# TaihuLight/Lol

Hardware: AMD Instinct MI355X
Metric: cyclotomic poly-muls/sec (CRT·pointwise·CRT⁻¹), batched; bit-exact vs CT (higher is better)
Workload: dtype u64

## Files before the change

lol_amd/csrc/pow2_impl.h:

```cpp
#pragma once
#include <hip/hip_runtime.h>

#include <atomic>
#include <mutex>
#include <type_traits>
#include <utility>

#include "kernels.h"
#include "zq_dev.h"

namespace lolhip {


constexpr int R = 4;
constexpr int E = 1 << R;
#ifndef LOLHIP_LEVEL_PARTS
#define LOLHIP_LEVEL_PARTS 4
#endif

#ifdef LOLHIP_STAMPS
static __device__ unsigned long long* g_stamp_buf = nullptr;
#define LH_STAMP(i) do { unsigned long long t_; asm volatile("s_memtime %0\n\ts_waitcnt lgkmcnt(0)" : "=s"(t_) :: "memory"); \
    if (g_stamp_buf && (threadIdx.x & 63) == 0) g_stamp_buf[((size_t)blockIdx.x * (blockDim.x >> 6) + (threadIdx.x >> 6)) * 32 + (i)] = t_; } while (0)
#else
// ... 53 lines not shown
    j += len;
  }
  return r;
}
template <Lay A, int I>
__device__ __forceinline__ int xthr_run(int tau) {
  constexpr LayRuns r = lay_runs(A);
  if constexpr (I < r.n) return (((tau >> r.src[I]) & ((1 << r.len[I]) - 1)) << r.dst[I]) | xthr_run<A, I + 1>(tau);
  else return 0;
}
template <Lay A>
__device__ __forceinline__ int xthr(int tau) { return xthr_run<A, 0>(tau); }

template <Lay A> struct LayTab {
  int xr[E];
  constexpr LayTab() : xr{} { for (int e = 0; e < E; ++e) xr[e] = xreg(A, e); }
};
template <Lay A> inline constexpr LayTab<A> lay_tab{};

constexpr int lpad(int x) { return x + (x >> 4); }

template <int AR> using VT = std::conditional_t<AR >= 2, u32, u64>;

struct QK {
  u64 q, nq, q2, nq2, q4, nq4;
  template <bool UNIFORM>
  __device__ __forceinline__ QK(const ModCtx& mc, std::bool_constant<UNIFORM> u) : QK(mc.q, u) {}
  template <bool UNIFORM>
  __device__ __forceinline__ QK(u64 q_, std::bool_constant<UNIFORM>) : q(q_), nq(0 - q_), q2(2 * q_), nq2(0 - 2 * q_), q4(4 * q_), nq4(0 - 4 * q_) {
    if constexpr (UNIFORM) asm volatile("" : "+s"(nq), "+s"(nq2), "+s"(nq4));
    else asm volatile("" : "+v"(nq), "+v"(nq2), "+v"(nq4));
  }
};
struct QK32 {
  u32 q, q2, mu;
  u32 r, rp, nqinv;
  template <bool UNIFORM>
  __device__ __forceinline__ QK32(const ModCtx& mc, std::bool_constant<UNIFORM>)
      : q((u32)mc.q), q2(2 * (u32)mc.q), mu((u32)(mc.mu >> 32)), r(mc.r32), rp(mc.r32p), nqinv((u32)mc.nqinv) {}
};
template <int AR> using QKT = std::conditional_t<AR >= 2, QK32, QK>;

__device__ __forceinline__ u32 csub32(u32 x, u32 m) { return min(x, x - m); }
__device__ __forceinline__ u32 shoup32(u32 y, u32 w, u32 wp, u32 q) { return w * y - __umulhi(wp, y) * q; }

#ifndef LOLHIP_PAIR_BFLY
#define LOLHIP_PAIR_BFLY 0
#endif
__device__ __forceinline__ u64 pair_of(u32 lo) { typedef u32 u32p __attribute__((ext_vector_type(2))); u32p t; t.x = lo; return __builtin_bit_cast(u64, t); }
template <bool WS>
__device__ __forceinline__ void fwd_pair(u32& X, u32& Y, u32 x, u32 w, u32 wp, u32 q, u32 q2) {
  const u64 xp = pair_of(x), q2p = (u64)q2;
  const u32 nq = 0u - q;
  u64 Xn, Z, Yn, cy; u32 Q;
#define LH_FWD_PAIR(WC)                                                                                     \
  asm("v_mul_hi_u32 %[Q], %[wp], %[yl]\n\t"                                                                  \
      "v_mad_u64_u32 %[Xn], %[cy], %[w], %[yl], %[X]\n\t"                                                    \
      "v_lshl_add_u64 %[Z], %[X], 1, %[q2]\n\t"                                                              \
      "v_mad_u64_u32 %[Xn], %[cy], %[Q], %[nq], %[Xn]"                                                        \
      : [Q] "=&v"(Q), [Xn] "=&v"(Xn), [Z] "=&v"(Z), [cy] "=&s"(cy)                                            \
      : [wp] WC(wp), [yl] "v"(Y), [w] WC(w), [X] "v"(xp), [q2] "s"(q2p), [nq] "s"(nq))
  if constexpr (WS) { LH_FWD_PAIR("s"); } else { LH_FWD_PAIR("v"); }
#undef LH_FWD_PAIR
  asm("v_mad_u64_u32 %[Yn], %[cy], %[xl], -1, %[Z]" : [Yn] "=v"(Yn), [cy] "=s"(cy) : [xl] "v"((u32)Xn), [Z] "v"(Z));
  X = (u32)Xn; Y = (u32)Yn;
}
template <bool WS>
__device__ __forceinline__ u32 shoup_pair(u32 d, u32 w, u32 wp, u32 q) {
  const u32 nq = 0u - q;
  const u32 Q = __umulhi(wp, d);
  u64 T, Yn, cy;
#define LH_SH_PAIR(WC)                                                                                      \
  asm("v_mad_u64_u32 %[T], %[cy], %[w], %[d], 0\n\t"                                                         \
      "v_mad_u64_u32 %[Yn], %[cy], %[Q], %[nq], %[T]"                                                         \
      : [T] "=&v"(T), [Yn] "=&v"(Yn), [cy] "=&s"(cy) : [w] WC(w), [d] "v"(d), [Q] "v"(Q), [nq] "s"(nq))
  if constexpr (WS) { LH_SH_PAIR("s"); } else { LH_SH_PAIR("v"); }
#undef LH_SH_PAIR
  return (u32)Yn;
}

template <int AR, bool WS = false, bool L1 = false>
__device__ __forceinline__ void bfly_fwd(VT<AR>& X, VT<AR>& Y, VT<AR> w, VT<AR> wp, const QKT<AR>& k) {
  if constexpr (AR == 3) {
    const u32 x = csub32(X, k.q);
    const u32 t = csub32(shoup32(Y, w, wp, k.q), k.q);
    X = x + t;
    Y = x - t + k.q;
  } else if constexpr (AR == 2) {
    const u32 x = csub32(X, k.q2);
#if LOLHIP_PAIR_BFLY
    fwd_pair<WS>(X, Y, x, w, wp, k.q, k.q2);
#else
    const u32 t = shoup32(Y, w, wp, k.q);
    X = x + t;
    Y = x - t + k.q2;
#endif
  } else if constexpr (AR == 4) {
#if LOLHIP_PAIR_BFLY
    fwd_pair<WS>(X, Y, X, w, wp, k.q, k.q2);
#else
    const u32 t = shoup32(Y, w, wp, k.q);
    const u32 x = X;
    X = x + t;
    Y = x - t + k.q2;
#endif
  } else if constexpr (AR == 1) {
#ifdef LH_ABL_NO_FWD_CSUB
    const u64 x = X;
#else
    const u64 x = L1 ? X : csubn(X, k.nq4);
#endif
    const u64 xn = shoup_acc<WS>(Y, w, wp, k.nq, x);
    const u64 z = shl1_add64u(x, k.q4);
    X = xn;
    Y = z - xn;
  } else {
    const u64 x = csub(X, k.q2);
    const u64 t = shoup_lazy(Y, w, wp, k.q);
    X = x + t;
    Y = x - t + k.q2;
  }
}
template <int AR, bool WS = false>
__device__ __forceinline__ void bfly_inv(VT<AR>& X, VT<AR>& Y, VT<AR> w, VT<AR> wp, const QKT<AR>& k) {
  if constexpr (AR == 3) {
    const u32 s = X + Y;
    const u32 d = X - Y + k.q;
    X = csub32(s, k.q);
    Y = csub32(shoup32(d, w, wp, k.q), k.q);
  } else if constexpr (AR == 2 || AR == 4) {
    const u32 s = X + Y;
    const u32 d = X - Y + k.q2;
    X = csub32(s, k.q2);
#if LOLHIP_PAIR_BFLY
    Y = shoup_pair<WS>(d, w, wp, k.q);
#else
    Y = shoup32(d, w, wp, k.q);
#endif
  } else if constexpr (AR == 1) {
    const u64 s = add64(X, Y);
    const u64 d = add64u(X, k.q4) - Y;
    X = csubn(s, k.nq4);
    Y = shoup_acc<WS>(d, w, wp, k.nq, 0);
  } else {
    const u64 s = X + Y;
    const u64 d = X - Y + k.q2;
    X = csub(s, k.q2);
    Y = shoup_lazy(d, w, wp, k.q);
  }
}
template <int AR, bool WS = false>
__device__ __forceinline__ void bfly_inv_last(VT<AR>& X, VT<AR>& Y, VT<AR> w, VT<AR> wp, VT<AR> s0, VT<AR> s1, const QKT<AR>& k) {
  if constexpr (AR == 3) {
    const u32 s = X + Y;
    const u32 d = X - Y + k.q;
    X = csub32(shoup32(s, s0, s1, k.q), k.q);
    Y = csub32(shoup32(d, w, wp, k.q), k.q);
  } else if constexpr (AR == 2 || AR == 4) {
    const u32 s = X + Y;
    const u32 d = X - Y + k.q2;
    X = shoup32(s, s0, s1, k.q);
    Y = shoup32(d, w, wp, k.q);
  } else if constexpr (AR == 1) {
    const u64 s = add64(X, Y);
    const u64 d = add64u(X, k.q4) - Y;
    X = shoup_acc<WS>(s, s0, s1, k.nq, 0);
    Y = shoup_acc<WS>(d, w, wp, k.nq, 0);
  } else {
    const u64 s = X + Y;
    const u64 d = X - Y + k.q2;
    X = shoup_lazy(s, s0, s1, k.q);
    Y = shoup_lazy(d, w, wp, k.q);
  }
}
template <int AR> __device__ __forceinline__ VT<AR> canon_fwd(VT<AR> v, const QKT<AR>& k) {
  if constexpr (AR == 3) return csub32(v, k.q);
  else if constexpr (AR == 2) return csub32(csub32(v, k.q2), k.q);
  else if constexpr (AR == 4) return csub32(v - __umulhi(v, k.mu) * k.q, k.q);
  else {
    if constexpr (AR == 1) v = csubn(v, k.nq4);
    return csubn(csubn(v, k.nq2), k.nq);
  }
}
template <int AR> __device__ __forceinline__ VT<AR> canon_inv(VT<AR> v, const QKT<AR>& k) {
  if constexpr (AR == 3) return v;
  else if constexpr (AR == 2 || AR == 4) return csub32(v, k.q);
  else {
    if constexpr (AR == 1) v = csubn(v, k.nq2);
    return csubn(v, k.nq);
  }
}
template <int AR> __device__ __forceinline__ VT<AR> from_i64(i64 x, const QKT<AR>& k) {
  if constexpr (AR >= 2) return (u32)x + (k.q & (u32)(x >> 63));
  else return canon_in(x, k.q);
}
template <int AR> __device__ __forceinline__ VT<AR> from_i64_fwd(i64 x, const QKT<AR>& k) {
  if constexpr (AR == 1) return add64u((u64)x, k.q);
  else if constexpr (AR >= 2) return (u32)x + k.q;
  else return from_i64<AR>(x, k);
}
template <int AR> __device__ __forceinline__ VT<AR> from_i64_inv(i64 x, const QKT<AR>& k) {
  if constexpr (AR == 1) return add64u((u64)x, k.q2);
  else if constexpr (AR == 2 || AR == 4) return (u32)x + k.q;
  else return from_i64<AR>(x, k);
}
template <int AR> __device__ __forceinline__ VT<AR> park_fwd(VT<AR> v, const QKT<AR>& k) {
  if constexpr (AR >= 2) return csub32(shoup32(v, k.r, k.rp, k.q), k.q);
  else if constexpr (AR == 1) return csubn(csubn(v, k.nq4), k.nq2);
  else return canon_fwd<AR>(v, k);
}
template <int AR> __device__ __forceinline__ VT<AR> pmul(VT<AR> a, VT<AR> b, const ModCtx& mc, const QKT<AR>& k) {
  if constexpr (AR >= 2) {
    const u64 x = (u64)a * b;
    const u32 m = (u32)x * k.nqinv;
    const u32 t = (u32)((x + (u64)m * k.q) >> 32);
    if constexpr (AR == 3) return csub32(t, k.q);
    else return t;
  } else if constexpr (AR == 1) {
#ifdef LOLHIP_ABL_PMUL
    return a + b;
#endif
    const unsigned __int128 T = (unsigned __int128)a * b;
    const u64 lo = (u64)T;
    return (u64)(T >> 64) + __umul64hi(lo * mc.nqinv, mc.q) + (lo != 0);
  } else {
    return mulmod(a, canon_fwd<0>(b, k), mc);
  }
}

typedef u32 u32x2 __attribute__((ext_vector_type(2)));
typedef u32 u32x4 __attribute__((ext_vector_type(4)));
typedef __amdgpu_buffer_rsrc_t rsrc_t;

__device__ __forceinline__ void load_tw(rsrc_t tw, u32 voff, u32 const_idx, u64& w, u64& wp) {
// ... 142 lines not shown
        load_tw(INV ? tw.inv : tw.fwd, voff, (u32)cidx, t.w[ord], t.wp[ord]);
      }
    }
    ++ord;
  }
}
template <int NT, typename V>
__device__ __forceinline__ void tw_fill_lds(V* dst, rsrc_t src, u32 comp, int n, int tau) {
  const int cnt = (n < TWL_HI ? n : TWL_HI) - TWL_LO;
  for (int i = tau; i < cnt; i += NT) {
    if constexpr (sizeof(V) == 8) {
      const u32x4 r = __builtin_amdgcn_raw_buffer_load_b128(src, comp + (u32)(TWL_LO + i) * 16u, 0, 0);
      *reinterpret_cast<u32x4*>(dst + 2 * i) = r;
    } else {
      const u32x2 r = __builtin_amdgcn_raw_buffer_load_b64(src, comp + (u32)(TWL_LO + i) * 8u, 0, 0);
      *reinterpret_cast<u32x2*>(dst + 2 * i) = r;
    }
  }
}
#ifndef LOLHIP_WS
#define LOLHIP_WS 1
#endif
template <int AR, bool INV, Lay A, int K, int HALF = -1>
__device__ __forceinline__ void level(VT<AR> (&v)[E], const LevelTwT<VT<AR>>& t, const TwCtxT<VT<AR>>& tw, const QKT<AR>& qk) {
  constexpr int beta = A.reg[K];
#ifdef LOLHIP_ABL_NO_BFLY
#pragma unroll
  for (int s = 0; s < 8; ++s) asm volatile("" :: "v"(t.w[s]), "v"(t.wp[s]));
  return;
#endif
  int ordb = -1;
#pragma unroll
  for (int e = 0; e < E; ++e) {
    if (e & (1 << K)) continue;
    ++ordb;
    if (HALF >= 0 && ordb / (8 / LOLHIP_LEVEL_PARTS) != HALF) continue;
    const int s = level_tab<A, K>.slot[e];
    constexpr bool WU = LOLHIP_WS && (A.ntb + R >= 10);
    if constexpr (!INV) bfly_fwd<AR, WU && tw_uniform<A, K>(), beta == 0>(v[e], v[e | (1 << K)], t.w[s], t.wp[s], qk);
    else if constexpr (beta == 0) bfly_inv_last<AR, WU>(v[e], v[e | (1 << K)], tw.l1w, tw.l1wp, tw.sc0, tw.sc1, qk);
    else bfly_inv<AR, WU && tw_uniform<A, K>()>(v[e], v[e | (1 << K)], t.w[s], t.wp[s], qk);
  }
}

template <int TB, int RK>
__device__ __forceinline__ void lane_swap(u32 (&v)[E]) {
  static_assert(TB == 4 || TB == 5, "only lane bits 4 and 5 have swap instructions");
// ... 86 lines not shown
  }
  static constexpr int G_K0 = R - (L - 10);
  static constexpr Lay io() {
    if (W16) {
      if (L < 10) { int thr[12] = {1, 2, 3, 4, 5, 6, 7, 8, 9, 10, 11, 12}; return lay_make(L, 0, L - 3, L - 2, L - 1, thr); }
      int thr[12] = {1, 2, 3, 4, 5, 6, 10, 11, 12, 13, 14, 15};
      return lay_make(L, 0, 7, 8, 9, thr);
    }
    if (L < 10) return lay_std(L, L - R);
    int thr[12] = {0, 1, 2, 3, 4, 5, 10, 11, 12, 13, 14, 15};
    return lay_make(L, 6, 7, 8, 9, thr);
  }
  static constexpr Lay final_layout() { return HAS_G ? g() : wave_end(); }
};

template <int AR, bool INV, Lay A, int K0, int K1 = R>
__device__ __forceinline__ void fetch4(LevelTwT<VT<AR>> (&t)[R], const TwCtxT<VT<AR>>& tw, int xt) {
  if constexpr (K0 <= 0 && K1 > 0) tw_fetch<INV, A, 0>(t[0], tw, xt);
  if constexpr (K0 <= 1 && K1 > 1) tw_fetch<INV, A, 1>(t[1], tw, xt);
  if constexpr (K0 <= 2 && K1 > 2) tw_fetch<INV, A, 2>(t[2], tw, xt);
  if constexpr (K0 <= 3 && K1 > 3) tw_fetch<INV, A, 3>(t[3], tw, xt);
}
template <int AR, bool INV, Lay A, int K>
__device__ __forceinline__ void level_jit(VT<AR> (&v)[E], const TwCtxT<VT<AR>>& tw, int xt, const QKT<AR>& qk) {
  using LevelTw = LevelTwT<VT<AR>>;
  if constexpr (tw_distinct(A, K) == 8 && sizeof(VT<AR>) == 8) {
    [&]<int... PART>(std::integer_sequence<int, PART...>) {
      (([&] { LevelTw t; tw_fetch<INV, A, K, PART>(t, tw, xt); level<AR, INV, A, K, PART>(v, t, tw, qk); }()), ...);
    }(std::make_integer_sequence<int, LOLHIP_LEVEL_PARTS>{});
  } else {
    LevelTw t; tw_fetch<INV, A, K>(t, tw, xt); level<AR, INV, A, K>(v, t, tw, qk);
  }
}
template <int AR, Lay A, int K0, int K1 = R>
__device__ __forceinline__ void levels4_jit(VT<AR> (&v)[E], const TwCtxT<VT<AR>>& tw, int xt, const QKT<AR>& qk) {
  if constexpr (K0 <= 0 && K1 > 0) level_jit<AR, false, A, 0>(v, tw, xt, qk);
  if constexpr (K0 <= 1 && K1 > 1) level_jit<AR, false, A, 1>(v, tw, xt, qk);
  if constexpr (K0 <= 2 && K1 > 2) level_jit<AR, false, A, 2>(v, tw, xt, qk);
  if constexpr (K0 <= 3 && K1 > 3) level_jit<AR, false, A, 3>(v, tw, xt, qk);
}
template <int AR, bool INV, Lay A, int K0, int K1 = R>
__device__ __forceinline__ void levels4(VT<AR> (&v)[E], const LevelTwT<VT<AR>> (&t)[R], const TwCtxT<VT<AR>>& tw, const QKT<AR>& qk) {
  if constexpr (!INV) {
    if constexpr (K0 <= 0 && K1 > 0) level<AR, false, A, 0>(v, t[0], tw, qk);
    if constexpr (K0 <= 1 && K1 > 1) level<AR, false, A, 1>(v, t[1], tw, qk);
    if constexpr (K0 <= 2 && K1 > 2) level<AR, false, A, 2>(v, t[2], tw, qk);
    if constexpr (K0 <= 3 && K1 > 3) level<AR, false, A, 3>(v, t[3], tw, qk);
  } else {
    if constexpr (K0 <= 3 && K1 > 3) level<AR, true, A, 3>(v, t[3], tw, qk);
    if constexpr (K0 <= 2 && K1 > 2) level<AR, true, A, 2>(v, t[2], tw, qk);
    if constexpr (K0 <= 1 && K1 > 1) level<AR, true, A, 1>(v, t[1], tw, qk);
    if constexpr (K0 <= 0 && K1 > 0) level<AR, true, A, 0>(v, t[0], tw, qk);
  }
}

__device__ __forceinline__ int fresh(int x) {
  asm volatile("" : "+v"(x));
  return x;
}

struct NoTop {};
template <int AR, int L, Lay PREV, int SB = 0, bool LEAN = false, bool W16 = false, typename TOP = NoTop, bool TRUNC = false>
__device__ __forceinline__ void fwd_transform(VT<AR> (&v)[E], VT<AR>* lds, const TwCtxT<VT<AR>>& tw, int tau_in, const QKT<AR>& qk,
                                              TOP* pre = nullptr) {
  constexpr bool PRE = !std::is_same_v<TOP, NoTop>;
  using LevelTw = LevelTwT<VT<AR>>;
  using S = Sched<L, W16>;
  static_assert(!TRUNC || (L >= 11 && !PRE), "the truncated forward transform needs the G layout");
  constexpr int GK1 = TRUNC ? 2 : R;
  constexpr bool L10 = !(TRUNC && L == 11);
  {
    constexpr Lay A = S::w0();
    const int tau = fresh(tau_in);
    if constexpr (S::HAS_G && !lay_eq(PREV, A)) __syncthreads();
    transpose_put<PREV, A, false>(v, lds, tau);
    if constexpr (LEAN) {
      transpose_get<PREV, A, false>(v, lds, tau);
      levels4_jit<AR, A, 0>(v, tw, xthr<A>(tau), qk);
    } else {
      LevelTw t[R];
      fetch4<AR, false, A, 0>(t, tw, xthr<A>(tau));
      transpose_get<PREV, A, false>(v, lds, tau);
      LH_STAMP(SB + 2);
      levels4<AR, false, A, 0>(v, t, tw, qk);
      LH_STAMP(SB + 3);
    }
// ... 39 lines not shown
    const int tau = fresh(tau_in);
    transpose_put<S::wave_end(), A, false>(v, lds, tau);
    if constexpr (PRE) {
      transpose_get<S::wave_end(), A, true>(v, lds, tau);
      LH_STAMP(SB + 7);
      pre->wait_g();
      levels4<AR, false, A, S::G_K0>(v, pre->g, tw, qk);
      LH_STAMP(SB + 8);
    } else if constexpr (LEAN) {
      transpose_get<S::wave_end(), A, true>(v, lds, tau);
      levels4_jit<AR, A, S::G_K0, GK1>(v, tw, xthr<A>(tau), qk);
    } else {
      LevelTw t[R];
      fetch4<AR, false, A, S::G_K0, GK1>(t, tw, xthr<A>(tau));
      transpose_get<S::wave_end(), A, true>(v, lds, tau);
      LH_STAMP(SB + 7);
      levels4<AR, false, A, S::G_K0, GK1>(v, t, tw, qk);
      LH_STAMP(SB + 8);
    }
  }
}

template <int AR, int L, Lay NEXT, bool W16 = false, bool TRUNC = false>
__device__ __forceinline__ void inv_transform(VT<AR> (&v)[E], VT<AR>* lds, const TwCtxT<VT<AR>>& tw, int tau_in, const QKT<AR>& qk) {
  using LevelTw = LevelTwT<VT<AR>>;
  using S = Sched<L, W16>;
  static_assert(!TRUNC || L >= 11, "the truncated inverse transform needs the G layout");
  constexpr int GK1 = TRUNC ? 2 : R;
  constexpr bool L10 = !(TRUNC && L == 11);
  if constexpr (S::HAS_G) {
    constexpr Lay A = S::g();
    const int tau = fresh(tau_in);
    LevelTw t[R];
    fetch4<AR, true, A, S::G_K0, GK1>(t, tw, xthr<A>(tau));
    levels4<AR, true, A, S::G_K0, GK1>(v, t, tw, qk);
    transpose_put<A, S::wave_end(), true>(v, lds, tau);
  }
  if constexpr (S::HAS_W1) {
    constexpr Lay A = S::w1();
    const int tau = fresh(tau_in);
    const int xt = xthr<A>(tau);
    LevelTw ua, ub, t[R];
    if constexpr (S::NSWAP >= 2 && L10) tw_fetch<true, S::w1b(), 2>(ub, tw, xthr<S::w1b()>(tau));
    if constexpr (S::NSWAP >= 1) tw_fetch<true, S::w1a(), 3>(ua, tw, xthr<S::w1a()>(tau));
    if constexpr (S::NSWAP == 0) fetch4<AR, true, A, S::W1_K0>(t, tw, xt);
    if constexpr (S::HAS_G) transpose_get<S::g(), S::wave_end(), true>(v, lds, tau);
    if constexpr (S::NSWAP >= 2) { if constexpr (L10) level<AR, true, S::w1b(), 2>(v, ub, tw, qk); lane_swap<5, 2>(v); }
// ... 52 lines not shown
        [y2l] "v"(lo32(y[2])), [y2h] "v"(hi32(y[2])), [y3l] "v"(lo32(y[3])), [y3h] "v"(hi32(y[3])));
}
__device__ __forceinline__ u64 dot4_redc(const u64 (&x)[4], const u64 (&y)[4], const ModCtx& mc) {
  u64 A, B1, B2, C;
  dot4_cols(x, y, A, B1, B2, C);
  const u64 u = (u64)hi32(C) + lo32(B1) + lo32(B2);
  const u64 lo = ((u64)lo32(u) << 32) | lo32(C);
  const u64 hi = A + hi32(B1) + hi32(B2) + hi32(u);
  return hi + __umul64hi(lo * mc.nqinv, mc.q) + (lo != 0);
}
template <Lay G>
__device__ __forceinline__ void pow2_base4(u64 (&v)[E], const u64 (&va)[E], const TwCtxT<u64>& tw, int xt, const ModCtx& mc, const QK& qk) {
  LevelTwT<u64> z;
  tw_fetch<false, G, 1>(z, tw, xt);
#pragma unroll
  for (int g = 0; g < 4; ++g) {
    constexpr int EK[4] = {0, 8, 4, 12};
    u64 zw = z.w[level_tab<G, 1>.slot[g & 1]], zwp = z.wp[level_tab<G, 1>.slot[g & 1]];
    if (g & 2) { zw = qk.q - zw; zwp = ~zwp; }
    u64 a[4], y[4];
#pragma unroll
    for (int k = 0; k < 4; ++k) {
      a[k] = va[g | EK[k]];
      y[k] = csubn(csubn(v[g | EK[k]], qk.nq4), qk.nq2);
    }
#pragma unroll
    for (int k = 3; k >= 0; --k) {
      u64 x[4], w[4];
#pragma unroll
      for (int i = 0; i < 4; ++i) { x[i] = a[i]; w[i] = y[(k - i) & 3]; }
      v[g | EK[k]] = dot4_redc(x, w, mc);
      asm volatile("" : "+v"(v[g | EK[k]]));
      if (k) y[k] = csubn(shoup_acc<false>(y[k], zw, zwp, qk.nq, 0), qk.nq2);
    }
  }
}

constexpr int pow2_threads(int L) { return (1 << (L - R)) >= 256 ? (1 << (L - R)) : 256; }

template <int L, int MODE, int AR, bool T1 = false, bool TR = false>
__global__ void __launch_bounds__(pow2_threads(L), AR >= 2 ? 8 : 4)
k_pow2(i64* y, const i64* a_in, const i64* b_in, i64 B, int T,
       const VT<AR>* __restrict__ tw_fwd, const VT<AR>* __restrict__ tw_inv, const VT<AR>* __restrict__ scale,
       const ModCtx* __restrict__ mod, int xcd_map) {
  using S = Sched<L, T1>;
  using V = VT<AR>;
  static_assert(!TR || (MODE == 2 && AR == 1 && L >= 11), "the truncated route is the 61-bit fused poly-mul's");
  constexpr int n = 1 << L;
  constexpr int NT = 1 << (L - R);
  constexpr int PPW = NT >= 256 ? 1 : 256 / NT;
  constexpr int LDSW = n + n / 16 + twl_words(n);
  constexpr u32 TWB = 2 * sizeof(V);
  extern __shared__ __attribute__((aligned(16))) unsigned char smem[];
  V* lds = reinterpret_cast<V*>(smem) + (threadIdx.x / NT) * LDSW;
  V* lds_tw = lds + n + n / 16;
  const int tau = threadIdx.x % NT;
  if constexpr (T1) T = 1;

  const i64 item0 = (i64)blockIdx.x * PPW;
  const int slot = (PPW == 1) ? 0 : (int)(threadIdx.x / NT);
  const i64 item = item0 + slot;
  i64 b, b0; int t;
  if (xcd_map) { i64 g = item / (8 * (i64)T); int r = (int)(item % (8 * T)); b = g * 8 + (r & 7); t = r >> 3; b0 = b; }
  else { b = item / T; t = (int)(item % T); b0 = item0 / T; }
  if constexpr (T1) { b = item; t = 0; b0 = item0; }

  if constexpr (NT >= 64) {
    t = __builtin_amdgcn_readfirstlane(t);
    b = (i64)(((u64)(u32)__builtin_amdgcn_readfirstlane((int)(b >> 32)) << 32) | (u32)__builtin_amdgcn_readfirstlane((int)b));
  }
  b0 = (i64)(((u64)(u32)__builtin_amdgcn_readfirstlane((int)(b0 >> 32)) << 32) | (u32)__builtin_amdgcn_readfirstlane((int)b0));
  const QKT<AR> qk(mod[t], std::bool_constant<(NT >= 64 || T1)>{});
  const u64 win = (u64)(B - b0) * n * T * 8;
  const u32 wbytes = win > 0xFFFFFFFFull ? 0xFFFFFFFFu : (u32)win;
  const size_t wbase = (size_t)b0 * n * T;
  const rsrc_t ry = __builtin_amdgcn_make_buffer_rsrc((void*)(y + wbase), 0, wbytes, 0x00020000);
  const rsrc_t ra = __builtin_amdgcn_make_buffer_rsrc((void*)(a_in + (MODE == 2 ? wbase : 0)), 0, MODE == 2 ? wbytes : 0, 0x00020000);
  const rsrc_t rb = __builtin_amdgcn_make_buffer_rsrc((void*)(b_in + (MODE == 2 ? wbase : 0)), 0, MODE == 2 ? wbytes : 0, 0x00020000);
  TwCtxT<V> tw;
  tw.fwd = __builtin_amdgcn_make_buffer_rsrc((void*)tw_fwd, 0, (u32)T * n * TWB, 0x00020000);
  tw.inv = __builtin_amdgcn_make_buffer_rsrc((void*)tw_inv, 0, (u32)T * n * TWB, 0x00020000);
  tw.comp = (u32)t * (u32)n * TWB;
  tw.pf = tw_fwd + (size_t)t * n * 2;
  tw.pi = tw_inv + (size_t)t * n * 2;
  tw.lds_tw = lds_tw;
  if constexpr (L >= TWL_MIN_L) tw_fill_lds<NT>(lds_tw, (MODE == 1) ? tw.inv : tw.fwd, tw.comp, n, tau);
  constexpr int SC = (MODE == 2 && AR == 1) ? 4 : 0;
  const V* scp = TR ? scale + (size_t)T * 8 + (size_t)t * 4 : scale + (size_t)t * 8 + SC;
  tw.sc0 = scp[0];
  tw.sc1 = scp[1];
  tw.l1w = scp[2];
  tw.l1wp = scp[3];

  constexpr Lay LIO = S::io();
  constexpr Lay LFIN = S::final_layout();
  const u32 uT8 = (u32)T * 8u;
  const u32 pofs = ((u32)(b - b0) * (u32)n * (u32)T + (u32)t) * 8u;
  const u32 off_io = pofs + (u32)xthr<LIO>(tau) * uT8;
  const u32 off_fin = pofs + (u32)xthr<LFIN>(tau) * uT8;

  V v[E];
  LH_STAMP(0);
#ifdef LOLHIP_STAMPS
  if (g_stamp_buf && (threadIdx.x & 63) == 0) {
    unsigned hwid, xcc;
    asm volatile("s_getreg_b32 %0, hwreg(HW_REG_HW_ID)" : "=s"(hwid));
    asm volatile("s_getreg_b32 %0, hwreg(HW_REG_XCC_ID)" : "=s"(xcc));
    g_stamp_buf[((size_t)blockIdx.x * (blockDim.x >> 6) + (threadIdx.x >> 6)) * 32 + 30] = ((unsigned long long)xcc << 32) | hwid;
  }
#endif
  if constexpr (MODE == 0 || MODE == 2) {
    const rsrc_t src = (MODE == 2) ? ra : ry;
    load_poly<LIO, T1>(src, off_io, uT8, [&](int e, u64 x) { v[e] = from_i64_fwd<AR>((i64)x, qk); });
    LH_STAMP(1);
    fwd_transform<AR, L, LIO, 0, false, T1, NoTop, TR>(v, lds, tw, tau, qk);
    if constexpr (MODE == 0) LH_STAMP(20);
  }
  if constexpr (MODE == 2) {
    V va[E];
#pragma unroll
    for (int e = 0; e < E; ++e) {
      va[e] = park_fwd<AR>(v[e], qk);
      if constexpr (TR) asm volatile("" : "+v"(va[e]));
    }
    LH_STAMP(9);
    const bool square = (a_in == b_in);
    if (!square) {
      u64 raw[E];
      load_poly<LIO, T1>(rb, off_io, uT8, [&](int e, u64 x) { raw[e] = x; });
      __builtin_amdgcn_sched_barrier(0);
#pragma unroll
      for (int e = 0; e < E; ++e) v[e] = from_i64_fwd<AR>((i64)raw[e], qk);
      LH_STAMP(11);
      fwd_transform<AR, L, LIO, 10, true, T1, NoTop, TR>(v, lds, tw, tau, qk);
    }
    LH_STAMP(19);
    const ModCtx mc = mod[t];
    if constexpr (TR) {
      pow2_base4<LFIN>(v, va, tw, xthr<LFIN>(fresh(tau)), mc, qk);
    } else {
#pragma unroll
      for (int e = 0; e < E; ++e) v[e] = pmul<AR>(va[e], (AR < 2 && square) ? va[e] : v[e], mc, qk);
    }
    LH_STAMP(22);
  }
  if constexpr (MODE == 2 && L >= TWL_MIN_L) {
    if constexpr (L > 10) __syncthreads();
    tw_fill_lds<NT>(lds_tw, tw.inv, tw.comp, n, tau);
  }
  if constexpr (MODE == 1) {
    load_poly<LFIN, T1>(ry, off_fin, uT8, [&](int e, u64 x) { v[e] = from_i64_inv<AR>((i64)x, qk); });
  }
  if constexpr (MODE == 0) {
    store_poly<LFIN, T1>(ry, off_fin, uT8, [&](int e) { return (u64)canon_fwd<AR>(v[e], qk); });
    LH_STAMP(21);
  } else {
    LH_STAMP(23);
    inv_transform<AR, L, LIO, T1, TR>(v, lds, tw, tau, qk);
    LH_STAMP(24);
    store_poly<LIO, T1>(ry, off_io, uT8, [&](int e) { return (u64)canon_inv<AR>(v[e], qk); });
    LH_STAMP(25);
  }
}

constexpr int MAX_DEV = 64;
struct KernelDev { std::atomic<int> state{0}; };
inline std::mutex& kernel_dev_mutex() { static std::mutex m; return m; }
template <typename Setup>
static hipError_t kernel_dev_setup(KernelDev (&tab)[MAX_DEV], Setup&& setup) {
  int dev = -1;
  hipError_t e = hipGetDevice(&dev);
  if (e != hipSuccess) return e;
  if (dev < 0 || dev >= MAX_DEV) return hipErrorInvalidDevice;
  KernelDev& d = tab[dev];
  if (d.state.load(std::memory_order_acquire) != 2) {
    std::lock_guard<std::mutex> g(kernel_dev_mutex());
    if (d.state.load(std::memory_order_relaxed) != 2) {
      e = setup();
      if (e != hipSuccess) return e;
      d.state.store(2, std::memory_order_release);
// ... 63 lines not shown
```

lol_amd/csrc/zq_dev.h:

```cpp
#pragma once
#include <stdint.h>

#if defined(__HIPCC__)
#include <hip/hip_runtime.h>
#define LH_HD __host__ __device__ __forceinline__
#define LH_D __device__ __forceinline__
#else
#define LH_HD inline
#define LH_D inline
#endif

namespace lolhip {

typedef uint64_t u64;
typedef uint32_t u32;
typedef int64_t i64;

struct ModCtx {
  u64 q;
  u64 d;
  u64 v;
  u32 s;
  u32 r32;
  u64 mu;
// ... 50 lines not shown

#ifndef LOLHIP_ASM_MAD
#define LOLHIP_ASM_MAD 3
#endif
LH_D u64 mad64(u32 a, u32 b, u64 c) {
#if LOLHIP_ASM_MAD
  u64 d, carry;
  asm("v_mad_u64_u32 %0, %1, %2, %3, %4" : "=v"(d), "=s"(carry) : "v"(a), "v"(b), "v"(c));
  return d;
#else
  return (u64)a * (u64)b + c;
#endif
}
LH_D u64 add64(u64 a, u64 b) { return a + b; }
LH_D u64 shl1_add64(u64 a, u64 b) { return (a << 1) + b; }
LH_D u64 add64u(u64 a, u64 b_uniform) { return a + b_uniform; }
LH_D u64 shl1_add64u(u64 a, u64 b_uniform) { return (a << 1) + b_uniform; }
LH_D u32 lo32(u64 x) { return (u32)x; }
LH_D u32 hi32(u64 x) { return (u32)(x >> 32); }

LH_D u64 csubn(u64 x, u64 negm) {
  u64 t = add64u(x, negm);
  return ((int)hi32(t) < 0) ? x : t;
}

template <bool WS = false>
LH_D u64 shoup_acc(u64 y, u64 w, u64 wp, u64 nq, u64 init) {
#if LOLHIP_ASM_MAD == 4
  u64 t = init, h, sj;
  asm("v_mad_u64_u32 v[120:121], vcc, %[wph], %[ylo], 0\n\t"
      "v_mad_u64_u32 v[120:121], vcc, %[wpl], %[yhi], v[120:121]\n\t"
      "v_mad_u64_u32 %[t], %[sj], %[wl], %[ylo], %[t]\n\t"
      "v_mad_u64_u32 %[h], %[sj], %[wl], %[yhi], 0\n\t"
      "v_mad_u64_u32 %[h], %[sj], %[wh], %[ylo], %[h]\n\t"
      "v_mov_b32 v122, v121\n\t"
      "v_cndmask_b32_e64 v123, 0, 1, vcc\n\t"
      "v_mad_u64_u32 v[118:119], %[sj], %[wph], %[yhi], v[122:123]\n\t"
      "v_mad_u64_u32 %[t], %[sj], v118, %[nql], %[t]\n\t"
      "v_mad_u64_u32 %[h], %[sj], v118, %[nqh], %[h]\n\t"
      "v_mad_u64_u32 %[h], %[sj], v119, %[nql], %[h]"
      : [t] "+v"(t), [h] "=&v"(h), [sj] "=&s"(sj)
      : [wph] "v"(hi32(wp)), [wpl] "v"(lo32(wp)), [ylo] "v"(lo32(y)), [yhi] "v"(hi32(y)),
        [wl] "v"(lo32(w)), [wh] "v"(hi32(w)), [nql] "s"(lo32(nq)), [nqh] "s"(hi32(nq))
      : "vcc", "v118", "v119", "v120", "v121", "v122", "v123");
  u32 th = hi32(t) + lo32(h);
  asm("" : "+v"(th));
// ... 32 lines not shown
  if constexpr (WS) { LH_SHOUP_BLOCKS(LH_WC_S); } else { LH_SHOUP_BLOCKS(LH_WC_V); }
#undef LH_SHOUP_BLOCKS
#undef LH_WC_V
#undef LH_WC_S
  u32 th = hi32(t) + lo32(h);
  asm("" : "+v"(th));
  return ((u64)th << 32) | lo32(t);
#else
  const u32 ah = __umulhi(hi32(wp), lo32(y));
  const u32 bh = __umulhi(lo32(wp), hi32(y));
  const u64 Q = mad64(bh, 1u, mad64(hi32(wp), hi32(y), (u64)ah));
  u64 t = mad64(lo32(w), lo32(y), init);
  t = mad64(lo32(Q), lo32(nq), t);
  u64 h = mad64(lo32(w), hi32(y), 0);
  h = mad64(hi32(w), lo32(y), h);
  h = mad64(lo32(Q), hi32(nq), h);
  h = mad64(hi32(Q), lo32(nq), h);
  u32 th = hi32(t) + lo32(h);
  asm("" : "+v"(th));
  return ((u64)th << 32) | lo32(t);
#endif
}

LH_D u64 rem128(u64 x1, u64 x0, const ModCtx& c) {
  u64 u1 = (x1 << c.s) | (x0 >> (64 - c.s));
  u64 u0 = x0 << c.s;
  unsigned __int128 qq = (unsigned __int128)c.v * u1 + (((unsigned __int128)u1 << 64) | u0);
  u64 q1 = (u64)(qq >> 64) + 1, q0 = (u64)qq;
  u64 r = u0 - q1 * c.d;
  if (r > q0) r += c.d;
  if (r >= c.d) r -= c.d;
  return r >> c.s;
}

LH_D u64 mulmod(u64 a, u64 b, const ModCtx& c) {
  unsigned __int128 z = (unsigned __int128)a * b;
  return rem128((u64)(z >> 64), (u64)z, c);
}

LH_D u64 reduce128(u64 x1, u64 x0, const ModCtx& c) {
  u64 r1 = rem128(0, x1, c);
  return rem128(r1, x0, c);
}

LH_D u64 addmod(u64 a, u64 b, u64 q) { u64 s = a + b; return s >= q ? s - q : s; }
LH_D u64 submod(u64 a, u64 b, u64 q) { return a >= b ? a - b : a + q - b; }
// ... 5 lines not shown
```

Before: 9.260 million.

## Use exec-masked conditional subtracts and defer per-modulus loads in tight mode

Adds csubx variants that perform 64-bit conditional subtraction with v_cmpx plus an exec-masked add, replacing the add/compare/select sequence in the radix-2 butterflies, canonicalisation and park steps when the modulus constants are wave-uniform. One of them is fused into the Shoup multiply asm block. For a small-thread-count pointwise mode, a new TIGHT path keeps per-lane constants unlaundered and defers loading inverse twiddle pointers and scale factors until the inverse transform, to cut live registers across the forward transform and pointwise stage. The cost is exec-mask manipulation with an s_nop pad and more template plumbing through auto-typed parameters.

```diff
diff --git a/lol_amd/csrc/pow2_impl.h b/lol_amd/csrc/pow2_impl.h
--- a/lol_amd/csrc/pow2_impl.h
+++ b/lol_amd/csrc/pow2_impl.h
@@ -99,16 +99,28 @@
 
 template <int AR> using VT = std::conditional_t<AR >= 2, u32, u64>;
 
-struct QK {
+template <bool UNIFORM, bool LAUNDER = true>
+struct QKx {
+  static constexpr bool uniform = UNIFORM;
   u64 q, nq, q2, nq2, q4, nq4;
-  template <bool UNIFORM>
-  __device__ __forceinline__ QK(const ModCtx& mc, std::bool_constant<UNIFORM> u) : QK(mc.q, u) {}
-  template <bool UNIFORM>
-  __device__ __forceinline__ QK(u64 q_, std::bool_constant<UNIFORM>) : q(q_), nq(0 - q_), q2(2 * q_), nq2(0 - 2 * q_), q4(4 * q_), nq4(0 - 4 * q_) {
+  __device__ __forceinline__ QKx(const ModCtx& mc, std::bool_constant<UNIFORM> u) : QKx(mc.q, u) {}
+  __device__ __forceinline__ QKx(u64 q_, std::bool_constant<UNIFORM>) : q(q_), nq(0 - q_), q2(2 * q_), nq2(0 - 2 * q_), q4(4 * q_), nq4(0 - 4 * q_) {
+    static_assert(LAUNDER || !UNIFORM, "only the per-lane constants may be left visible");
     if constexpr (UNIFORM) asm volatile("" : "+s"(nq), "+s"(nq2), "+s"(nq4));
-    else asm volatile("" : "+v"(nq), "+v"(nq2), "+v"(nq4));
+    else if constexpr (LAUNDER) asm volatile("" : "+v"(nq), "+v"(nq2), "+v"(nq4));
   }
 };
+typedef QKx<true> QK;
+template <class K> inline constexpr bool trim_exec = LOLHIP_CSUB_EXEC && std::remove_cvref_t<K>::uniform;
+template <bool U, bool LD> __device__ __forceinline__ u64 trim2(u64 v, const QKx<U, LD>& k) {
+  if constexpr (trim_exec<QKx<U, LD>>) return csubx(v, k.q2, k.nq2); else return csubn(v, k.nq2);
+}
+template <bool U, bool LD> __device__ __forceinline__ u64 trim42(u64 v, const QKx<U, LD>& k) {
+  if constexpr (trim_exec<QKx<U, LD>>) return csubx2(v, k.q4, k.nq4, k.q2, k.nq2); else return csubn(csubn(v, k.nq4), k.nq2);
+}
+template <bool U, bool LD> __device__ __forceinline__ u64 trim21(u64 v, const QKx<U, LD>& k) {
+  if constexpr (trim_exec<QKx<U, LD>>) return csubx2(v, k.q2, k.nq2, k.q, k.nq); else return csubn(csubn(v, k.nq2), k.nq);
+}
 struct QK32 {
   u32 q, q2, mu;
   u32 r, rp, nqinv;
@@ -116,7 +128,7 @@
   __device__ __forceinline__ QK32(const ModCtx& mc, std::bool_constant<UNIFORM>)
       : q((u32)mc.q), q2(2 * (u32)mc.q), mu((u32)(mc.mu >> 32)), r(mc.r32), rp(mc.r32p), nqinv((u32)mc.nqinv) {}
 };
-template <int AR> using QKT = std::conditional_t<AR >= 2, QK32, QK>;
+template <int AR, bool UNIFORM = true, bool LAUNDER = true> using QKT = std::conditional_t<AR >= 2, QK32, QKx<UNIFORM, LAUNDER>>;
 
 __device__ __forceinline__ u32 csub32(u32 x, u32 m) { return min(x, x - m); }
 __device__ __forceinline__ u32 shoup32(u32 y, u32 w, u32 wp, u32 q) { return w * y - __umulhi(wp, y) * q; }
@@ -157,7 +169,7 @@
 }
 
 template <int AR, bool WS = false, bool L1 = false>
-__device__ __forceinline__ void bfly_fwd(VT<AR>& X, VT<AR>& Y, VT<AR> w, VT<AR> wp, const QKT<AR>& k) {
+__device__ __forceinline__ void bfly_fwd(VT<AR>& X, VT<AR>& Y, VT<AR> w, VT<AR> wp, const auto& k) {
   if constexpr (AR == 3) {
     const u32 x = csub32(X, k.q);
     const u32 t = csub32(shoup32(Y, w, wp, k.q), k.q);
@@ -184,10 +196,13 @@
   } else if constexpr (AR == 1) {
 #ifdef LH_ABL_NO_FWD_CSUB
     const u64 x = X;
+    const u64 xn = shoup_acc<WS>(Y, w, wp, k.nq, x);
 #else
-    const u64 x = L1 ? X : csubn(X, k.nq4);
-#endif
-    const u64 xn = shoup_acc<WS>(Y, w, wp, k.nq, x);
+    u64 x = X, xn;
+    if constexpr (L1) xn = shoup_acc<WS>(Y, w, wp, k.nq, x);
+    else if constexpr (trim_exec<decltype(k)>) xn = shoup_acc_csubx<WS, true>(Y, w, wp, k.nq, x, k.q4, k.nq4);
+    else { x = csubn(X, k.nq4); xn = shoup_acc<WS>(Y, w, wp, k.nq, x); }
+#endif
     const u64 z = shl1_add64u(x, k.q4);
     X = xn;
     Y = z - xn;
@@ -199,7 +214,7 @@
   }
 }
 template <int AR, bool WS = false>
-__device__ __forceinline__ void bfly_inv(VT<AR>& X, VT<AR>& Y, VT<AR> w, VT<AR> wp, const QKT<AR>& k) {
+__device__ __forceinline__ void bfly_inv(VT<AR>& X, VT<AR>& Y, VT<AR> w, VT<AR> wp, const auto& k) {
   if constexpr (AR == 3) {
     const u32 s = X + Y;
     const u32 d = X - Y + k.q;
@@ -217,8 +232,8 @@
   } else if constexpr (AR == 1) {
     const u64 s = add64(X, Y);
     const u64 d = add64u(X, k.q4) - Y;
-    X = csubn(s, k.nq4);
-    Y = shoup_acc<WS>(d, w, wp, k.nq, 0);
+    if constexpr (trim_exec<decltype(k)>) { X = s; Y = shoup_acc_csubx<WS, false>(d, w, wp, k.nq, X, k.q4, k.nq4); }
+    else { X = csubn(s, k.nq4); Y = shoup_acc<WS>(d, w, wp, k.nq, 0); }
   } else {
     const u64 s = X + Y;
     const u64 d = X - Y + k.q2;
@@ -227,7 +242,7 @@
   }
 }
 template <int AR, bool WS = false>
-__device__ __forceinline__ void bfly_inv_last(VT<AR>& X, VT<AR>& Y, VT<AR> w, VT<AR> wp, VT<AR> s0, VT<AR> s1, const QKT<AR>& k) {
+__device__ __forceinline__ void bfly_inv_last(VT<AR>& X, VT<AR>& Y, VT<AR> w, VT<AR> wp, VT<AR> s0, VT<AR> s1, const auto& k) {
   if constexpr (AR == 3) {
     const u32 s = X + Y;
     const u32 d = X - Y + k.q;
@@ -250,7 +265,7 @@
     Y = shoup_lazy(d, w, wp, k.q);
   }
 }
-template <int AR> __device__ __forceinline__ VT<AR> canon_fwd(VT<AR> v, const QKT<AR>& k) {
+template <int AR> __device__ __forceinline__ VT<AR> canon_fwd(VT<AR> v, const auto& k) {
   if constexpr (AR == 3) return csub32(v, k.q);
   else if constexpr (AR == 2) return csub32(csub32(v, k.q2), k.q);
   else if constexpr (AR == 4) return csub32(v - __umulhi(v, k.mu) * k.q, k.q);
@@ -259,34 +274,34 @@
     return csubn(csubn(v, k.nq2), k.nq);
   }
 }
-template <int AR> __device__ __forceinline__ VT<AR> canon_inv(VT<AR> v, const QKT<AR>& k) {
+template <int AR> __device__ __forceinline__ VT<AR> canon_inv(VT<AR> v, const auto& k) {
   if constexpr (AR == 3) return v;
   else if constexpr (AR == 2 || AR == 4) return csub32(v, k.q);
   else {
-    if constexpr (AR == 1) v = csubn(v, k.nq2);
-    return csubn(v, k.nq);
-  }
-}
-template <int AR> __device__ __forceinline__ VT<AR> from_i64(i64 x, const QKT<AR>& k) {
+    if constexpr (AR == 1) return trim21(v, k);
+    else return csubn(v, k.nq);
+  }
+}
+template <int AR> __device__ __forceinline__ VT<AR> from_i64(i64 x, const auto& k) {
   if constexpr (AR >= 2) return (u32)x + (k.q & (u32)(x >> 63));
   else return canon_in(x, k.q);
 }
-template <int AR> __device__ __forceinline__ VT<AR> from_i64_fwd(i64 x, const QKT<AR>& k) {
+template <int AR> __device__ __forceinline__ VT<AR> from_i64_fwd(i64 x, const auto& k) {
   if constexpr (AR == 1) return add64u((u64)x, k.q);
   else if constexpr (AR >= 2) return (u32)x + k.q;
   else return from_i64<AR>(x, k);
 }
-template <int AR> __device__ __forceinline__ VT<AR> from_i64_inv(i64 x, const QKT<AR>& k) {
+template <int AR> __device__ __forceinline__ VT<AR> from_i64_inv(i64 x, const auto& k) {
   if constexpr (AR == 1) return add64u((u64)x, k.q2);
   else if constexpr (AR == 2 || AR == 4) return (u32)x + k.q;
   else return from_i64<AR>(x, k);
 }
-template <int AR> __device__ __forceinline__ VT<AR> park_fwd(VT<AR> v, const QKT<AR>& k) {
+template <int AR> __device__ __forceinline__ VT<AR> park_fwd(VT<AR> v, const auto& k) {
   if constexpr (AR >= 2) return csub32(shoup32(v, k.r, k.rp, k.q), k.q);
-  else if constexpr (AR == 1) return csubn(csubn(v, k.nq4), k.nq2);
+  else if constexpr (AR == 1) return trim42(v, k);
   else return canon_fwd<AR>(v, k);
 }
-template <int AR> __device__ __forceinline__ VT<AR> pmul(VT<AR> a, VT<AR> b, const ModCtx& mc, const QKT<AR>& k) {
+template <int AR> __device__ __forceinline__ VT<AR> pmul(VT<AR> a, VT<AR> b, const ModCtx& mc, const auto& k) {
   if constexpr (AR >= 2) {
     const u64 x = (u64)a * b;
     const u32 m = (u32)x * k.nqinv;
@@ -475,7 +490,7 @@
 #define LOLHIP_WS 1
 #endif
 template <int AR, bool INV, Lay A, int K, int HALF = -1>
-__device__ __forceinline__ void level(VT<AR> (&v)[E], const LevelTwT<VT<AR>>& t, const TwCtxT<VT<AR>>& tw, const QKT<AR>& qk) {
+__device__ __forceinline__ void level(VT<AR> (&v)[E], const LevelTwT<VT<AR>>& t, const TwCtxT<VT<AR>>& tw, const auto& qk) {
   constexpr int beta = A.reg[K];
 #ifdef LOLHIP_ABL_NO_BFLY
 #pragma unroll
@@ -608,7 +623,7 @@
   if constexpr (K0 <= 3 && K1 > 3) tw_fetch<INV, A, 3>(t[3], tw, xt);
 }
 template <int AR, bool INV, Lay A, int K>
-__device__ __forceinline__ void level_jit(VT<AR> (&v)[E], const TwCtxT<VT<AR>>& tw, int xt, const QKT<AR>& qk) {
+__device__ __forceinline__ void level_jit(VT<AR> (&v)[E], const TwCtxT<VT<AR>>& tw, int xt, const auto& qk) {
   using LevelTw = LevelTwT<VT<AR>>;
   if constexpr (tw_distinct(A, K) == 8 && sizeof(VT<AR>) == 8) {
     [&]<int... PART>(std::integer_sequence<int, PART...>) {
@@ -619,14 +634,14 @@
   }
 }
 template <int AR, Lay A, int K0, int K1 = R>
-__device__ __forceinline__ void levels4_jit(VT<AR> (&v)[E], const TwCtxT<VT<AR>>& tw, int xt, const QKT<AR>& qk) {
+__device__ __forceinline__ void levels4_jit(VT<AR> (&v)[E], const TwCtxT<VT<AR>>& tw, int xt, const auto& qk) {
   if constexpr (K0 <= 0 && K1 > 0) level_jit<AR, false, A, 0>(v, tw, xt, qk);
   if constexpr (K0 <= 1 && K1 > 1) level_jit<AR, false, A, 1>(v, tw, xt, qk);
   if constexpr (K0 <= 2 && K1 > 2) level_jit<AR, false, A, 2>(v, tw, xt, qk);
   if constexpr (K0 <= 3 && K1 > 3) level_jit<AR, false, A, 3>(v, tw, xt, qk);
 }
 template <int AR, bool INV, Lay A, int K0, int K1 = R>
-__device__ __forceinline__ void levels4(VT<AR> (&v)[E], const LevelTwT<VT<AR>> (&t)[R], const TwCtxT<VT<AR>>& tw, const QKT<AR>& qk) {
+__device__ __forceinline__ void levels4(VT<AR> (&v)[E], const LevelTwT<VT<AR>> (&t)[R], const TwCtxT<VT<AR>>& tw, const auto& qk) {
   if constexpr (!INV) {
     if constexpr (K0 <= 0 && K1 > 0) level<AR, false, A, 0>(v, t[0], tw, qk);
     if constexpr (K0 <= 1 && K1 > 1) level<AR, false, A, 1>(v, t[1], tw, qk);
@@ -647,7 +662,7 @@
 
 struct NoTop {};
 template <int AR, int L, Lay PREV, int SB = 0, bool LEAN = false, bool W16 = false, typename TOP = NoTop, bool TRUNC = false>
-__device__ __forceinline__ void fwd_transform(VT<AR> (&v)[E], VT<AR>* lds, const TwCtxT<VT<AR>>& tw, int tau_in, const QKT<AR>& qk,
+__device__ __forceinline__ void fwd_transform(VT<AR> (&v)[E], VT<AR>* lds, const TwCtxT<VT<AR>>& tw, int tau_in, const auto& qk,
                                               TOP* pre = nullptr) {
   constexpr bool PRE = !std::is_same_v<TOP, NoTop>;
   using LevelTw = LevelTwT<VT<AR>>;
@@ -733,7 +748,7 @@
 }
 
 template <int AR, int L, Lay NEXT, bool W16 = false, bool TRUNC = false>
-__device__ __forceinline__ void inv_transform(VT<AR> (&v)[E], VT<AR>* lds, const TwCtxT<VT<AR>>& tw, int tau_in, const QKT<AR>& qk) {
+__device__ __forceinline__ void inv_transform(VT<AR> (&v)[E], VT<AR>* lds, const TwCtxT<VT<AR>>& tw, int tau_in, const auto& qk) {
   using LevelTw = LevelTwT<VT<AR>>;
   using S = Sched<L, W16>;
   static_assert(!TRUNC || L >= 11, "the truncated inverse transform needs the G layout");
@@ -832,7 +847,7 @@
 #pragma unroll
     for (int k = 0; k < 4; ++k) {
       a[k] = va[g | EK[k]];
-      y[k] = csubn(csubn(v[g | EK[k]], qk.nq4), qk.nq2);
+      y[k] = trim42(v[g | EK[k]], qk);
     }
 #pragma unroll
     for (int k = 3; k >= 0; --k) {
@@ -841,7 +856,7 @@
       for (int i = 0; i < 4; ++i) { x[i] = a[i]; w[i] = y[(k - i) & 3]; }
       v[g | EK[k]] = dot4_redc(x, w, mc);
       asm volatile("" : "+v"(v[g | EK[k]]));
-      if (k) y[k] = csubn(shoup_acc<false>(y[k], zw, zwp, qk.nq, 0), qk.nq2);
+      if (k) y[k] = trim2(shoup_acc<false>(y[k], zw, zwp, qk.nq, 0), qk);
     }
   }
 }
@@ -880,7 +895,8 @@
     b = (i64)(((u64)(u32)__builtin_amdgcn_readfirstlane((int)(b >> 32)) << 32) | (u32)__builtin_amdgcn_readfirstlane((int)b));
   }
   b0 = (i64)(((u64)(u32)__builtin_amdgcn_readfirstlane((int)(b0 >> 32)) << 32) | (u32)__builtin_amdgcn_readfirstlane((int)b0));
-  const QKT<AR> qk(mod[t], std::bool_constant<(NT >= 64 || T1)>{});
+  constexpr bool TIGHT = (AR == 1 && MODE == 2 && !(NT >= 64 || T1) && L >= 5);
+  const QKT<AR, (NT >= 64 || T1), !TIGHT> qk(mod[t], std::bool_constant<(NT >= 64 || T1)>{});
   const u64 win = (u64)(B - b0) * n * T * 8;
   const u32 wbytes = win > 0xFFFFFFFFull ? 0xFFFFFFFFu : (u32)win;
   const size_t wbase = (size_t)b0 * n * T;
@@ -892,15 +908,17 @@
   tw.inv = __builtin_amdgcn_make_buffer_rsrc((void*)tw_inv, 0, (u32)T * n * TWB, 0x00020000);
   tw.comp = (u32)t * (u32)n * TWB;
   tw.pf = tw_fwd + (size_t)t * n * 2;
-  tw.pi = tw_inv + (size_t)t * n * 2;
+  if constexpr (!TIGHT) tw.pi = tw_inv + (size_t)t * n * 2;
   tw.lds_tw = lds_tw;
   if constexpr (L >= TWL_MIN_L) tw_fill_lds<NT>(lds_tw, (MODE == 1) ? tw.inv : tw.fwd, tw.comp, n, tau);
   constexpr int SC = (MODE == 2 && AR == 1) ? 4 : 0;
   const V* scp = TR ? scale + (size_t)T * 8 + (size_t)t * 4 : scale + (size_t)t * 8 + SC;
-  tw.sc0 = scp[0];
-  tw.sc1 = scp[1];
-  tw.l1w = scp[2];
-  tw.l1wp = scp[3];
+  if constexpr (!TIGHT) {
+    tw.sc0 = scp[0];
+    tw.sc1 = scp[1];
+    tw.l1w = scp[2];
+    tw.l1wp = scp[3];
+  }
 
   constexpr Lay LIO = S::io();
   constexpr Lay LFIN = S::final_layout();
@@ -923,7 +941,7 @@
     const rsrc_t src = (MODE == 2) ? ra : ry;
     load_poly<LIO, T1>(src, off_io, uT8, [&](int e, u64 x) { v[e] = from_i64_fwd<AR>((i64)x, qk); });
     LH_STAMP(1);
-    fwd_transform<AR, L, LIO, 0, false, T1, NoTop, TR>(v, lds, tw, tau, qk);
+    fwd_transform<AR, L, LIO, 0, TIGHT, T1, NoTop, TR>(v, lds, tw, tau, qk);
     if constexpr (MODE == 0) LH_STAMP(20);
   }
   if constexpr (MODE == 2) {
@@ -945,7 +963,8 @@
       fwd_transform<AR, L, LIO, 10, true, T1, NoTop, TR>(v, lds, tw, tau, qk);
     }
     LH_STAMP(19);
-    const ModCtx mc = mod[t];
+    const int tl = TIGHT ? fresh(t) : t;
+    const ModCtx mc = mod[tl];
     if constexpr (TR) {
       pow2_base4<LFIN>(v, va, tw, xthr<LFIN>(fresh(tau)), mc, qk);
     } else {
@@ -966,6 +985,15 @@
     LH_STAMP(21);
   } else {
     LH_STAMP(23);
+    if constexpr (TIGHT) {
+      const int tl = fresh(t);
+      tw.pi = tw_inv + (size_t)tl * n * 2;
+      const V* sc = scale + (size_t)tl * 8 + SC;
+      tw.sc0 = sc[0];
+      tw.sc1 = sc[1];
+      tw.l1w = sc[2];
+      tw.l1wp = sc[3];
+    }
     inv_transform<AR, L, LIO, T1, TR>(v, lds, tw, tau, qk);
     LH_STAMP(24);
     store_poly<LIO, T1>(ry, off_io, uT8, [&](int e) { return (u64)canon_inv<AR>(v[e], qk); });
diff --git a/lol_amd/csrc/zq_dev.h b/lol_amd/csrc/zq_dev.h
--- a/lol_amd/csrc/zq_dev.h
+++ b/lol_amd/csrc/zq_dev.h
@@ -96,6 +96,50 @@
 LH_D u64 csubn(u64 x, u64 negm) {
   u64 t = add64u(x, negm);
   return ((int)hi32(t) < 0) ? x : t;
+}
+
+#ifndef LOLHIP_CSUB_EXEC
+#define LOLHIP_CSUB_EXEC 1
+#endif
+#ifndef LOLHIP_CSUBX_PAD
+#define LOLHIP_CSUBX_PAD 1
+#endif
+#if LOLHIP_CSUBX_PAD
+#define LH_CSUBX_TAIL "\n\ts_nop 1"
+#else
+#define LH_CSUBX_TAIL ""
+#endif
+#define LH_CSUBX(x, sv, m, nm)                                                                       \
+  "s_mov_b64 %[" sv "], exec\n\t"                                                                     \
+  "v_cmpx_ge_u64 vcc, %[" x "], %[" m "]\n\t"                                                         \
+  "v_lshl_add_u64 %[" x "], %[" x "], 0, %[" nm "]\n\t"                                                \
+  "s_mov_b64 exec, %[" sv "]"
+#define LH_CSUBX_SAVED(x, sv, m, nm)                                                                 \
+  "v_cmpx_ge_u64 vcc, %[" x "], %[" m "]\n\t"                                                         \
+  "v_lshl_add_u64 %[" x "], %[" x "], 0, %[" nm "]\n\t"                                                \
+  "s_mov_b64 exec, %[" sv "]"
+LH_D u64 csubx(u64 x, u64 m, u64 negm) {
+  u64 sv;
+  asm(LH_CSUBX("x", "sv", "m", "nm") LH_CSUBX_TAIL
+      : [x] "+v"(x), [sv] "=&s"(sv) : [m] "s"(m), [nm] "s"(negm) : "vcc");
+  return x;
+}
+LH_D u64 exec_save() {
+  u64 sv;
+  asm volatile("s_mov_b64 %0, exec" : "=s"(sv));
+  return sv;
+}
+LH_D u64 csubx(u64 x, u64 m, u64 negm, u64 saved_exec) {
+  asm(LH_CSUBX_SAVED("x", "sv", "m", "nm") LH_CSUBX_TAIL
+      : [x] "+v"(x) : [sv] "s"(saved_exec), [m] "s"(m), [nm] "s"(negm) : "vcc");
+  return x;
+}
+LH_D u64 csubx2(u64 x, u64 m1, u64 negm1, u64 m2, u64 negm2) {
+  u64 sv;
+  asm(LH_CSUBX("x", "sv", "m1", "nm1") "\n\t"
+      LH_CSUBX_SAVED("x", "sv", "m2", "nm2") LH_CSUBX_TAIL
+      : [x] "+v"(x), [sv] "=&s"(sv) : [m1] "s"(m1), [nm1] "s"(negm1), [m2] "s"(m2), [nm2] "s"(negm2) : "vcc");
+  return x;
 }
 
 template <bool WS = false>
@@ -174,6 +218,43 @@
 #endif
 }
 
+template <bool WS, bool INIT_X>
+LH_D u64 shoup_acc_csubx(u64 y, u64 w, u64 wp, u64 nq, u64& x, u64 m, u64 negm) {
+#if LOLHIP_ASM_MAD == 3
+  u64 Q, t, h, sv;
+  u32 ah, bh;
+#define LH_SHOUP_BLOCKS_X(WC)                                                                        \
+  asm(LH_CSUBX("x", "sv", "m", "nm") "\n\t"                                                          \
+      "v_mul_hi_u32 %[ah], %[wph], %[yl]\n\t"                                                        \
+      "v_mul_hi_u32 %[bh], %[wpl], %[yh]\n\t"                                                        \
+      "v_mad_u64_u32 %[Q], vcc, %[wph], %[yh], 0\n\t"                                                \
+      "v_mad_u64_u32 %[Q], vcc, %[ah], 1, %[Q]\n\t"                                                  \
+      "v_mad_u64_u32 %[Q], vcc, %[bh], 1, %[Q]"                                                      \
+      : [Q] "=&v"(Q), [ah] "=&v"(ah), [bh] "=&v"(bh), [x] "+v"(x), [sv] "=&s"(sv)                    \
+      : [wph] WC(hi32(wp)), [wpl] WC(lo32(wp)), [yl] "v"(lo32(y)), [yh] "v"(hi32(y)),                \
+        [m] "s"(m), [nm] "s"(negm)                                                                   \
+      : "vcc");                                                                                      \
+  asm("v_mad_u64_u32 %0, vcc, %2, %4, %10\n\t"                                                       \
+      "v_mad_u64_u32 %1, vcc, %2, %5, 0\n\t"                                                         \
+      "v_mad_u64_u32 %0, vcc, %6, %8, %0\n\t"                                                        \
+      "v_mad_u64_u32 %1, vcc, %3, %4, %1\n\t"                                                        \
+      "v_mad_u64_u32 %1, vcc, %6, %9, %1\n\t"                                                        \
+      "v_mad_u64_u32 %1, vcc, %7, %8, %1"                                                            \
+      : "=&v"(t), "=&v"(h)                                                                           \
+      : WC(lo32(w)), WC(hi32(w)), "v"(lo32(y)), "v"(hi32(y)), "v"(lo32(Q)), "v"(hi32(Q)),            \
+        "s"(lo32(nq)), "s"(hi32(nq)), "v"(INIT_X ? x : (u64)0)                                       \
+      : "vcc")
+  if constexpr (WS) { LH_SHOUP_BLOCKS_X("s"); } else { LH_SHOUP_BLOCKS_X("v"); }
+#undef LH_SHOUP_BLOCKS_X
+  u32 th = hi32(t) + lo32(h);
+  asm("" : "+v"(th));
+  return ((u64)th << 32) | lo32(t);
+#else
+  x = csubx(x, m, negm);
+  return shoup_acc<WS>(y, w, wp, nq, INIT_X ? x : (u64)0);
+#endif
+}
+
 LH_D u64 rem128(u64 x1, u64 x0, const ModCtx& c) {
   u64 u1 = (x1 << c.s) | (x0 >> (64 - c.s));
   u64 u0 = x0 << c.s;
```

After: 9.787 million, median of 6. +5.7%, better.
